# OSU-NLP-Group/saev

Hardware: AMD Instinct MI355X
Metric: activations/sec (train step), d_in=1024 x32 k=32 (higher is better)
Workload: dtype f32 (encoder: fp16 MFMA first pass with a rigorous error margin, survivors recomputed exactly in fp32; all else fp32)

## Files before the change

### saev_amd/csrc/common.h

```cpp
#pragma once
#include <hip/hip_runtime.h>
#include <stdint.h>

#define WAVE 64

typedef float f32x4 __attribute__((ext_vector_type(4)));
typedef float f32x16 __attribute__((ext_vector_type(16)));

__device__ __forceinline__ int32_t f2key(float f) {
    int32_t b = __float_as_int(f);
    return b >= 0 ? b : (b ^ 0x7fffffff);
}
__device__ __forceinline__ float key2f(int32_t k) {
    return __int_as_float(k >= 0 ? k : (k ^ 0x7fffffff));
}
__device__ __forceinline__ uint32_t f2ukey(float f) {
    uint32_t b = __float_as_uint(f);
    return (b & 0x80000000u) ? ~b : (b | 0x80000000u);
}
__device__ __forceinline__ float ukey2f(uint32_t k) {
    return __uint_as_float((k & 0x80000000u) ? (k & 0x7fffffffu) : ~k);
}

__device__ __forceinline__ float wave_sum(float v) {
#pragma unroll
    for (int o = 32; o > 0; o >>= 1) v += __shfl_xor(v, o, 64);
    return v;
}
__device__ __forceinline__ double wave_sum_d(double v) {
#pragma unroll
    for (int o = 32; o > 0; o >>= 1) v += __shfl_xor(v, o, 64);
    return v;
}
__device__ __forceinline__ int wave_sum_i(int v) {
#pragma unroll
    for (int o = 32; o > 0; o >>= 1) v += __shfl_xor(v, o, 64);
    return v;
}
__device__ __forceinline__ float wave_max(float v) {
#pragma unroll
    for (int o = 32; o > 0; o >>= 1) v = fmaxf(v, __shfl_xor(v, o, 64));
    return v;
}

#define NEG_INF (-__builtin_huge_valf())

__device__ __forceinline__ float rpg_apply(float g, float sc, float w) { return __builtin_fmaf(-sc, w, g); }
template <int NV>
__device__ __forceinline__ float rpg_row_stats(const f32x4 (&g)[NV], const f32x4 (&w)[NV], int project, float* sc_out) {
    float dot = 0.f, nsq = 0.f;
#pragma unroll
    for (int n = 0; n < NV; ++n)
#pragma unroll
        for (int e = 0; e < 4; ++e) { dot = __builtin_fmaf(g[n][e], w[n][e], dot); nsq = __builtin_fmaf(w[n][e], w[n][e], nsq); }
    dot = wave_sum(dot);
    nsq = wave_sum(nsq);
    const float sc = (project && nsq > 0.f) ? dot / nsq : 0.f;
    float sq = 0.f;
#pragma unroll
    for (int n = 0; n < NV; ++n)
#pragma unroll
        for (int e = 0; e < 4; ++e) { const float t = rpg_apply(g[n][e], sc, w[n][e]); sq = __builtin_fmaf(t, t, sq); }
    *sc_out = sc;
    return wave_sum(sq);
}
```

### saev_amd/csrc/sparse.hip

```cpp
#include "common.h"
#include "kernels.h"

namespace {

template <int NV>
__device__ __forceinline__ void gather_rows_accum(f32x4 (&acc)[NV], const float* __restrict__ W, int D, int D4,
                                                  const int32_t* idx_row, const float* val_row, int k, int limit,
                                                  int lane) {
    for (int j0 = 0; j0 < k; j0 += 64) {
        const int cnt = min(64, k - j0);
        int32_t my_i = -1;
        float my_v = 0.f;
        if (lane < cnt) { my_i = idx_row[j0 + lane]; my_v = val_row[j0 + lane]; }
#pragma unroll 4
        for (int jj = 0; jj < cnt; ++jj) {
            const int32_t i = __shfl(my_i, jj, 64);
            const float v = __shfl(my_v, jj, 64);
            if (i < 0 || i >= limit) continue;
            const f32x4* wr = reinterpret_cast<const f32x4*>(W + (size_t)i * D);
#pragma unroll
            for (int n = 0; n < NV; ++n) {
                const int q = lane + 64 * n;
                if (q < D4) {
                    const f32x4 w = wr[q];
// ... 544 lines not shown
    __syncthreads();
    int off[3] = {0, 0, 0};
    for (int j = 0; j < w; ++j)
        for (int q = 0; q < 3; ++q) off[q] += wave_tot[j][q];
    if (i < a.S) {
        a.starts[i] = off[0] + incl[0] - v[0];
        if (a.chunk_starts) {
            a.chunk_starts[i] = off[1] + incl[1] - v[1];
            a.part_starts[i] = off[2] + incl[2] - v[2];
        }
    }
    if (tid == 1023)
        for (int q = 0; q < 3; ++q) a.scan_totals[blockIdx.x * 3 + q] = off[q] + incl[q];
}
__global__ __launch_bounds__(1024) void csc_scan_offset_kernel(CscArgs a) {
    if (a.k_dev && *a.k_dev <= 0) return;
    __shared__ int base[3];
    const int tid = threadIdx.x, lane = tid & 63;
    if (tid < 64) {
        int s3[3] = {0, 0, 0};
        for (int b = lane; b < (int)blockIdx.x; b += 64)
            for (int q = 0; q < 3; ++q) s3[q] += a.scan_totals[b * 3 + q];
        for (int q = 0; q < 3; ++q) s3[q] = wave_sum_i(s3[q]);
        if (lane == 0)
            for (int q = 0; q < 3; ++q) base[q] = s3[q];
    }
    __syncthreads();
    const int i = blockIdx.x * 1024 + tid;
    if (i < a.S) {
        a.starts[i] += base[0];
        if (a.chunk_starts) { a.chunk_starts[i] += base[1]; a.part_starts[i] += base[2]; }
    }
    if (blockIdx.x == gridDim.x - 1 && tid == 0) {
        if (a.zero_word != nullptr) *a.zero_word = 0;
        a.starts[a.S] = base[0] + a.scan_totals[blockIdx.x * 3 + 0];
        if (a.chunk_starts) a.chunk_starts[a.S] = base[1] + a.scan_totals[blockIdx.x * 3 + 1];
    }
}

__global__ void csc_place_kernel(CscArgs a) {
    const int k = a.k_dev ? min(*a.k_dev, a.k) : a.k;
    if (k <= 0) return;
    const long n = (long)a.n_rows * k;
    const int groups = a.words >> 3;
    for (long p = (long)blockIdx.x * blockDim.x + threadIdx.x; p < max(n, (long)a.S); p += (long)gridDim.x * blockDim.x) {
        if (p < a.S && a.chunk_starts) {
            const int c1 = a.chunk_starts[p + 1];
            for (int c = a.chunk_starts[p]; c < c1; ++c) a.work_latent[c] = (int)p;
        }
        if (p >= n) continue;
        const int b = (int)(p / k), j = (int)(p % k);
        const int32_t i = a.idx[(size_t)b * a.code_stride + j];
        if (i < 0 || i >= a.S) continue;
        const int g = b >> 8, wi = (b >> 5) & 7;
        const uint4* grp = reinterpret_cast<const uint4*>(a.bitmap + (size_t)i * a.words + 8 * g);
        const uint4 lo = grp[0], hi = grp[1];
        const uint32_t wd[8] = {lo.x, lo.y, lo.z, lo.w, hi.x, hi.y, hi.z, hi.w};
        int rank = a.grp_prefix[(size_t)i * groups + g];
#pragma unroll
        for (int e = 0; e < 8; ++e) {
            const uint32_t m = e < wi ? 0xffffffffu : (e == wi ? ((1u << (b & 31)) - 1u) : 0u);
            rank += __popc(wd[e] & m);
        }
        const int slot = a.starts[i] + rank;
        if (a.pairs != nullptr) a.pairs[slot] = int2{b, (int)((size_t)b * a.code_stride + j)};
        if (a.pv != nullptr) {
            const int fl = (rank == 0 ? DWS_FIRST : 0) | (rank == a.counts[i] - 1 ? DWS_LAST : 0);
            int pblk = 0;
            if (a.P > 1) while (pblk < a.P - 1 && i >= a.cuts[pblk]) ++pblk;
            a.pv[slot] = int2{((pblk * a.n_rows + b) << 7) | fl, __float_as_int(a.val[(size_t)b * a.code_stride + j])};
            a.plat[slot] = i;
            if (a.pv2 != nullptr) a.pv2[slot] = int2{(b << 7) | fl, __float_as_int(a.dval[(size_t)b * a.code_stride + j])};
        }
    }
}


template <int NV>
__device__ __forceinline__ void write_row_proj(float2* row_proj, int i, const f32x4 (&g)[NV], const f32x4 (&w)[NV], int project,
                                               int lane) {
    float sc;
    const float sq = rpg_row_stats<NV>(g, w, project, &sc);
    if (lane == 0) row_proj[i] = float2{sc, sq};
}

template <int NV>
__device__ __forceinline__ float row_sumsq(const f32x4 (&g)[NV]) {
    float sq = 0.f;
#pragma unroll
    for (int n = 0; n < NV; ++n)
#pragma unroll
        for (int e = 0; e < 4; ++e) sq = __builtin_fmaf(g[n][e], g[n][e], sq);
    return wave_sum(sq);
}

#ifndef DW_MIN_WAVES
#define DW_MIN_WAVES 1
#endif
#ifndef DW_GROUP
#define DW_GROUP 8
#endif
template <int NV>
__global__ __launch_bounds__(256, DW_MIN_WAVES) void dw_rows_kernel(DwRowsArgs a) {
    if (a.k_dev && *a.k_dev <= 0) return;
    const int lane = threadIdx.x & 63;
    const int wi = a.chunk_starts[a.lat_lo] + blockIdx.x * 4 + (threadIdx.x >> 6);
    const int n_work = a.chunk_starts[a.lat_hi];
    if (wi >= n_work) return;
    const int i = a.work_latent[wi];
    const int c = wi - a.chunk_starts[i];
    const int nch = a.chunk_starts[i + 1] - a.chunk_starts[i];
    const int D = a.D, D4 = D >> 2;
    const int seg_beg = a.starts[i], seg_end = a.starts[i + 1];
    int pblk = 0;
    if (a.P > 1) while (pblk < a.P - 1 && i >= a.cuts[pblk]) ++pblk;
    const size_t g_stride = (size_t)a.P * D;
    const float* gbase = a.g + (size_t)pblk * D;
    const int beg = seg_beg + c * DW_CHUNK;
    const int end = min(seg_end, beg + DW_CHUNK);
    f32x4 accd[NV], acce[NV], wv[NV];
    {
        const f32x4* wr = reinterpret_cast<const f32x4*>(a.W_dec + (size_t)i * D);
#pragma unroll
        for (int n = 0; n < NV; ++n) {
            accd[n] = f32x4{0.f, 0.f, 0.f, 0.f};
            acce[n] = f32x4{0.f, 0.f, 0.f, 0.f};
            wv[n] = (a.part != 2 && lane + 64 * n < D4) ? wr[lane + 64 * n] : f32x4{0.f, 0.f, 0.f, 0.f};
        }
    }
    int my_b = 0;
    float my_v = 0.f, my_dv = 0.f;
    const int cnt = end - beg;
    const int part = a.part;
    if (lane < cnt) {
        const int2 pr = a.pairs[beg + lane];
        my_b = pr.x;
        my_v = a.val[pr.y];
        if (part == 2) my_dv = a.dval[beg + lane];
        if (a.clear_bitmap != nullptr) a.clear_bitmap[(size_t)i * a.clear_words + (my_b >> 5)] = 0u;
    }
    float dbs = 0.f;
    constexpr int G = DW_GROUP, GS = (G == 8 ? 3 : 4);
    for (int j0 = 0; j0 < cnt; j0 += G) {
        float p[G];
        float r = 0.f;
        if (part != 2) {
#pragma unroll
        for (int t = 0; t < G; t += 2) {
            p[t] = 0.f; p[t + 1] = 0.f;
            if (j0 + t >= cnt) continue;
            const bool two = j0 + t + 1 < cnt;
            const int b0 = __shfl(my_b, j0 + t, 64), b1 = __shfl(my_b, min(j0 + t + 1, 63), 64);
            const float v0 = __shfl(my_v, j0 + t, 64), v1 = two ? __shfl(my_v, min(j0 + t + 1, 63), 64) : 0.f;
            const f32x4* g0 = reinterpret_cast<const f32x4*>(gbase + (size_t)b0 * g_stride);
            const f32x4* g1 = reinterpret_cast<const f32x4*>(gbase + (size_t)(two ? b1 : b0) * g_stride);
            f32x4 tg0[NV], tg1[NV];
#pragma unroll
            for (int n = 0; n < NV; ++n) {
                const int q = lane + 64 * n;
                const bool ok = q < D4;
                tg0[n] = ok ? g0[q] : f32x4{0.f, 0.f, 0.f, 0.f};
                tg1[n] = ok ? g1[q] : f32x4{0.f, 0.f, 0.f, 0.f};
            }
#pragma unroll
            for (int n = 0; n < NV; ++n) {
                accd[n] += v0 * tg0[n];
                accd[n] += v1 * tg1[n];
                p[t] += tg0[n][0] * wv[n][0] + tg0[n][1] * wv[n][1] + tg0[n][2] * wv[n][2] + tg0[n][3] * wv[n][3];
                p[t + 1] += tg1[n][0] * wv[n][0] + tg1[n][1] * wv[n][1] + tg1[n][2] * wv[n][2] + tg1[n][3] * wv[n][3];
            }
            if (!two) p[t + 1] = 0.f;
        }
        r = wave_reduce_scatter<G>(p, lane);
        if (part == 1) {
            if ((lane & ((1 << GS) - 1)) == 0 && j0 + (lane >> GS) < cnt) a.dval[beg + j0 + (lane >> GS)] = r;
            continue;
        }
        }
#pragma unroll
        for (int t = 0; t < G; t += 2) {
            if (j0 + t >= cnt) continue;
            const bool two = j0 + t + 1 < cnt;
            const float e0 = part == 2 ? __shfl(my_dv, j0 + t, 64) : __shfl(r, t << GS, 64);
            const float e1 = !two ? 0.f : part == 2 ? __shfl(my_dv, min(j0 + t + 1, 63), 64) : __shfl(r, (t + 1) << GS, 64);
            dbs += e0 + e1;
            const int b0 = __shfl(my_b, j0 + t, 64), b1 = __shfl(my_b, min(j0 + t + 1, 63), 64);
            const f32x4* x0 = reinterpret_cast<const f32x4*>(a.x + (size_t)b0 * D);
            const f32x4* x1 = reinterpret_cast<const f32x4*>(a.x + (size_t)(two ? b1 : b0) * D);
            f32x4 tx0[NV], tx1[NV];
#pragma unroll
            for (int n = 0; n < NV; ++n) {
                const int q = lane + 64 * n;
                const bool ok = q < D4;
                tx0[n] = ok ? x0[q] : f32x4{0.f, 0.f, 0.f, 0.f};
                tx1[n] = ok ? x1[q] : f32x4{0.f, 0.f, 0.f, 0.f};
            }
#pragma unroll
            for (int n = 0; n < NV; ++n) {
                acce[n] += e0 * tx0[n];
                acce[n] += e1 * tx1[n];
            }
        }
    }

    float *od, *oe;
    bool direct = (nch == 1);
    if (direct) {
        od = a.dW_dec + (size_t)i * D;
        oe = a.dW_encT + (size_t)i * D;
    } else {
        od = a.partials + (size_t)(a.part_starts[i] + c) * 2 * D;
        oe = od + D;
    }
#pragma unroll
    for (int n = 0; n < NV; ++n) {
        const int q = lane + 64 * n;
        if (q < D4) {
            f32x4* pd = reinterpret_cast<f32x4*>(od) + q;
            f32x4* pe = reinterpret_cast<f32x4*>(oe) + q;
            if (part != 2) { if (direct && a.accumulate) *pd = *pd + accd[n]; else *pd = accd[n]; }
            if (part != 1) { if (direct && a.accumulate) *pe = *pe + acce[n]; else *pe = acce[n]; }
        }
    }
    if (lane == 0 && part != 1) {
        if (direct) a.db_enc[i] = a.accumulate ? (a.db_enc[i] + dbs) : dbs;
        else a.db_partials[a.part_starts[i] + c] = dbs;
    }
    if (a.row_proj != nullptr && direct && part != 2 && !a.accumulate) write_row_proj<NV>(a.row_proj, i, accd, wv, a.project, lane);
    if (a.enc_sq != nullptr && direct && part != 1 && !a.accumulate) {
        const float sq = row_sumsq<NV>(acce);
        if (lane == 0) a.enc_sq[i] = sq;
    }
}

template <int NV>
__global__ __launch_bounds__(256) void dw_combine_kernel(DwRowsArgs a) {
    if (a.k_dev && *a.k_dev <= 0) return;
    const int lane = threadIdx.x & 63;
    const int i = a.lat_lo + blockIdx.x * 4 + (threadIdx.x >> 6);
    if (i >= a.lat_hi) return;
    const int enc = blockIdx.y;
    if ((enc == 0 && a.part == 2) || (enc == 1 && a.part == 1)) return;
    const int nch = a.chunk_starts[i + 1] - a.chunk_starts[i];
    if (nch <= 1) return;
    const int c0 = a.part_starts[i], c1 = c0 + nch;
    const int D = a.D, D4 = D >> 2;
    const float* base = a.partials + (enc ? D : 0);
    f32x4 acc[NV];
#pragma unroll
    for (int n = 0; n < NV; ++n) acc[n] = f32x4{0.f, 0.f, 0.f, 0.f};
    float dbs = 0.f;
    int c = c0;
    constexpr int TRIP = NV <= 4 ? 8 : (NV <= 8 ? 4 : 2);
    for (; c + TRIP <= c1; c += TRIP) {
        f32x4 t[TRIP][NV];
#pragma unroll
        for (int u = 0; u < TRIP; ++u) {
            const f32x4* p = reinterpret_cast<const f32x4*>(base + (size_t)(c + u) * 2 * D);
#pragma unroll
            for (int n = 0; n < NV; ++n) t[u][n] = (lane + 64 * n < D4) ? p[lane + 64 * n] : f32x4{0.f, 0.f, 0.f, 0.f};
        }
#pragma unroll
        for (int n = 0; n < NV; ++n) {
            if constexpr (TRIP == 8) acc[n] += ((t[0][n] + t[1][n]) + (t[2][n] + t[3][n])) + ((t[4][n] + t[5][n]) + (t[6][n] + t[7][n]));
            else if constexpr (TRIP == 4) acc[n] += (t[0][n] + t[1][n]) + (t[2][n] + t[3][n]);
            else acc[n] += t[0][n] + t[1][n];
        }
        if (enc) {
#pragma unroll
            for (int u = 0; u < TRIP; ++u) dbs += a.db_partials[c + u];
        }
    }
    for (; c < c1; ++c) {
        const f32x4* p = reinterpret_cast<const f32x4*>(base + (size_t)c * 2 * D);
#pragma unroll
        for (int n = 0; n < NV; ++n)
            if (lane + 64 * n < D4) acc[n] += p[lane + 64 * n];
        if (enc) dbs += a.db_partials[c];
    }
    f32x4* o = reinterpret_cast<f32x4*>((enc ? a.dW_encT : a.dW_dec) + (size_t)i * D);
#pragma unroll
    for (int n = 0; n < NV; ++n) {
        const int q = lane + 64 * n;
        if (q < D4) o[q] = a.accumulate ? o[q] + acc[n] : acc[n];
    }
    if (enc) {
        if (lane == 0) a.db_enc[i] = a.accumulate ? (a.db_enc[i] + dbs) : dbs;
        if (a.enc_sq != nullptr && !a.accumulate) {
            const float sq = row_sumsq<NV>(acc);
            if (lane == 0) a.enc_sq[i] = sq;
        }
    } else if (a.row_proj != nullptr && !a.accumulate) {
        f32x4 wv[NV];
        const f32x4* wr = reinterpret_cast<const f32x4*>(a.W_dec + (size_t)i * D);
#pragma unroll
        for (int n = 0; n < NV; ++n) wv[n] = (lane + 64 * n < D4) ? wr[lane + 64 * n] : f32x4{0.f, 0.f, 0.f, 0.f};
        write_row_proj<NV>(a.row_proj, i, acc, wv, a.project, lane);
    }
}


typedef int i32x2 __attribute__((ext_vector_type(2)));
typedef int i32x4 __attribute__((ext_vector_type(4)));

__device__ __forceinline__ f32x4 buf_load16(__amdgpu_buffer_rsrc_t r, uint32_t voff) {
    const i32x4 v = __builtin_amdgcn_raw_buffer_load_b128(r, voff, 0, 0);
    return f32x4{__int_as_float(v[0]), __int_as_float(v[1]), __int_as_float(v[2]), __int_as_float(v[3])};
}
__device__ __forceinline__ float group8_sum(float v) {
    v += __int_as_float(__builtin_amdgcn_mov_dpp(__float_as_int(v), 0xB1, 0xF, 0xF, true));
    v += __int_as_float(__builtin_amdgcn_mov_dpp(__float_as_int(v), 0x4E, 0xF, 0xF, true));
    v += __int_as_float(__builtin_amdgcn_mov_dpp(__float_as_int(v), 0x141, 0xF, 0xF, true));
    return v;
}

__global__ __launch_bounds__(256) void slice_major_copy_kernel(const float* __restrict__ g, const float* __restrict__ x, int n, int D,
                                                               float* __restrict__ gS, float* __restrict__ xS) {
    const int lane = threadIdx.x & 63;
    const int row = blockIdx.x * 4 + (threadIdx.x >> 6);
    if (row >= n) return;
    const f32x4* gr = reinterpret_cast<const f32x4*>(g + (size_t)row * D);
    const f32x4* xr = reinterpret_cast<const f32x4*>(x + (size_t)row * D);
    for (int q = lane; q < (D >> 2); q += 64) {
        const size_t o = ((size_t)(q >> 3) * n + row) * 8 + (q & 7);
        reinterpret_cast<f32x4*>(gS)[o] = gr[q];
        reinterpret_cast<f32x4*>(xS)[o] = xr[q];
    }
}

template <bool DEC, bool DVAL = true>
__global__ __launch_bounds__(256, (DEC && DVAL) ? 4 : 5) void dw_slices_kernel(DwSlicesArgs a, int wg_per_slice) {
    constexpr bool PASS_A = DEC && DVAL;
    constexpr int L = DWS_RUN;
    const int lane = threadIdx.x & 63, gi = lane >> 3, li = lane & 7;
    const int xcd = blockIdx.x & 7, q = blockIdx.x >> 3;
    const int slice = xcd + 8 * (q / wg_per_slice);
    const bool sq_on = (DEC ? a.sq_wave_dec : a.sq_wave_enc) != nullptr;
    auto sq_slot = [&]() -> float* {
        return (DEC ? a.sq_wave_dec : a.sq_wave_enc) + ((size_t)blockIdx.x * 4 + __builtin_amdgcn_readfirstlane((int)(threadIdx.x >> 6)));
    };
    if (slice * DWS_SLICE >= a.D) { if (sq_on && lane == 0) *sq_slot() = 0.f; return; }
    const int NP = a.starts[a.S];
    const int run0 = ((q % wg_per_slice) * 4 + (threadIdx.x >> 6)) * 8;
    if (run0 * L >= NP) { if (sq_on && lane == 0) *sq_slot() = 0.f; return; }
    const int run = run0 + gi;
    const int col = slice * DWS_SLICE + li * 4;
    const uint32_t colb = (uint32_t)col * 4u, rowb = (uint32_t)a.D * 4u, li16 = (uint32_t)li * 16u;
    auto bound = [&](int r) -> int {
        const long nb = (long)r * L;
        if (nb >= NP) return NP;
        const int lat = a.plat[nb];
        const int s = a.starts[lat];
        return (a.starts[lat + 1] - s < L) ? s : (int)nb;
    };
    const int p0 = bound(run), p1 = bound(run + 1);
    const bool live = p0 < p1;
    const int2* const pv = DEC ? a.pv : a.pv2;
    float* const out = DEC ? a.dW_dec : a.dW_encT;
    float* const part = DEC ? a.part_dec : a.part_enc;
    f32x4 acc = {0.f, 0.f, 0.f, 0.f};
    f32x4 w4 = {0.f, 0.f, 0.f, 0.f};
    float* const dvp = PASS_A ? a.dvp + (size_t)slice * a.pair_cap : nullptr;
    __shared__ float sh_sq[256];
    sh_sq[threadIdx.x] = 0.f;
    const int sel = (lane & 56) << 2;
    const __amdgpu_buffer_rsrc_t mres = __builtin_amdgcn_make_buffer_rsrc(
        const_cast<float*>(DEC ? a.gS : a.xS) + (size_t)slice * a.n_rows * DWS_SLICE * (DEC && a.P > 1 ? a.P : 1), 0,
        (uint32_t)a.n_rows * 128u * (uint32_t)(DEC && a.P > 1 ? a.P : 1), 0x00020000);
    const __amdgpu_buffer_rsrc_t wres = __builtin_amdgcn_make_buffer_rsrc(const_cast<float*>(a.W_dec), 0, (uint32_t)a.S * rowb, 0x00020000);

    auto load_info = [&](int t, int2& e, int& lat) {
        const int p = p0 + 8 * t + li;
        e = int2{0, 0};
        lat = 0;
        if (p < p1) {
            const i32x2 v = reinterpret_cast<const i32x2*>(pv)[p];
            e = int2{v[0], v[1]};
            lat = a.plat[p];
            if (p == p1 - 1) e.x |= DWS_END;
            if (p == p0) e.x &= ~DWS_FIRST;
        }
    };
    constexpr int PB = 4;
    auto issue = [&](const int2& e, int lat, int j0, int (&xj)[PB], int (&lj)[PB], f32x4 (&gt)[PB], f32x4 (&wt)[PB]) {
#pragma unroll
        for (int j = 0; j < PB; ++j) {
            xj[j] = __builtin_amdgcn_ds_bpermute(sel + 4 * (j0 + j), e.x);
            lj[j] = __builtin_amdgcn_ds_bpermute(sel + 4 * (j0 + j), lat);
            gt[j] = buf_load16(mres, ((uint32_t)xj[j] & ~127u) | li16);
            if (PASS_A && (xj[j] & DWS_FIRST)) wt[j] = buf_load16(wres, (uint32_t)lj[j] * rowb + colb);
        }
    };
    auto consume = [&](const int2& e, int j0, const int (&xc)[PB], const int (&lc)[PB], const f32x4 (&gc)[PB], const f32x4 (&wc)[PB],
                       const f32x4& wnext0, bool& head_open, float& dmine) {
        float vc[PB];
#pragma unroll
        for (int j = 0; j < PB; ++j) vc[j] = __int_as_float(__builtin_amdgcn_ds_bpermute(sel + 4 * (j0 + j), e.y));
#pragma unroll
        for (int j = 0; j < PB; ++j) {
            if (PASS_A) {
                float d = gc[j][0] * w4[0] + gc[j][1] * w4[1] + gc[j][2] * w4[2] + gc[j][3] * w4[3];
                d = group8_sum(d);
                dmine = li == j0 + j ? d : dmine;
            }
            acc += vc[j] * gc[j];
            if (xc[j] & (DWS_LAST | DWS_END)) {
                float* o;
                if (head_open) o = part + ((size_t)run * 2 + 0) * a.D + col;
                else if (!(xc[j] & DWS_LAST)) o = part + ((size_t)run * 2 + 1) * a.D + col;
                else {
                    o = out + (size_t)lc[j] * a.D + col;
                    if (sq_on)
                        sh_sq[threadIdx.x] += __builtin_fmaf(acc[3], acc[3], __builtin_fmaf(acc[2], acc[2], __builtin_fmaf(acc[1], acc[1], acc[0] * acc[0])));
                }
                *reinterpret_cast<f32x4*>(o) = acc;
                if (DEC && slice == 0 && li == 0 && (xc[j] & DWS_END)) {
                    const int cl = (!head_open && !(xc[j] & DWS_LAST)) ? lc[j] : -1;
                    a.cut_lat[run] = cl;
                    if (cl >= 0 && a.cut_list != nullptr)
                        reinterpret_cast<i32x4*>(a.cut_list)[1 + atomicAdd(&a.cut_list[0], 1)] = i32x4{run, cl, a.starts[cl], a.starts[cl + 1]};
                }
                head_open = false;
                acc = f32x4{0.f, 0.f, 0.f, 0.f};
                if (PASS_A) w4 = j + 1 < PB ? wc[j + 1 < PB ? j + 1 : 0] : wnext0;
            }
        }
    };
    int2 e_c, e_n;
    int lat_c, lat_n;
    int xa[PB], xb[PB], la[PB], lb[PB];
    f32x4 ga[PB], gb[PB], wa[PB], wb[PB];
    bool head_open = false;
    load_info(0, e_c, lat_c);
    if (live) {
        head_open = (pv[p0].x & DWS_FIRST) == 0;
        if (PASS_A) w4 = buf_load16(wres, (uint32_t)a.plat[p0] * rowb + colb);
    }
    issue(e_c, lat_c, 0, xa, la, ga, wa);
    load_info(1, e_n, lat_n);
#pragma unroll 1
    for (int t = 0; __any(p0 + 8 * t < p1); ++t) {
        float dmine = 0.f;
        issue(e_c, lat_c, PB, xb, lb, gb, wb);
        consume(e_c, 0, xa, la, ga, wa, wb[0], head_open, dmine);
        issue(e_n, lat_n, 0, xa, la, ga, wa);
        consume(e_c, PB, xb, lb, gb, wb, wa[0], head_open, dmine);
        if (PASS_A && p0 + 8 * t + li < p1) dvp[p0 + 8 * t + li] = dmine;
        e_c = e_n; lat_c = lat_n;
        load_info(t + 2, e_n, lat_n);
    }
    if (sq_on) {
        const float sq = wave_sum(sh_sq[threadIdx.x]);
        if (lane == 0) *sq_slot() = sq;
    }
}

__global__ __launch_bounds__(256) void dw_dval_sum_kernel(DwSlicesArgs a) {
    const int NP = a.starts[a.S];
    const int p = blockIdx.x * 256 + threadIdx.x;
    if (p >= NP) return;
    const int n_slices = a.D / DWS_SLICE;
    float s = 0.f;
    for (int c = 0; c < n_slices; ++c) s += a.dvp[(size_t)c * a.pair_cap + p];
    const int2 e = a.pv[p];
    const int b = a.P > 1 ? (e.x >> 7) % a.n_rows : (e.x >> 7);
    a.pv2[p] = int2{(b << 7) | (e.x & 127), __float_as_int(s)};
    if (a.clear_bitmap != nullptr) a.clear_bitmap[(size_t)a.plat[p] * a.clear_words + (b >> 5)] = 0u;
}

__global__ __launch_bounds__(256) void dw_clear_bitmap_kernel(DwSlicesArgs a) {
    const int NP = a.starts[a.S];
    const int p = blockIdx.x * 256 + threadIdx.x;
    if (p >= NP) return;
    a.clear_bitmap[(size_t)a.plat[p] * a.clear_words + (a.pv2[p].x >> 12)] = 0u;
}

template <int NV>
__global__ __launch_bounds__(256) void dw_finalize_cut_kernel(DwSlicesArgs a, int kind0) {
    constexpr int L = DWS_RUN;
    __shared__ f32x4 sh[3][NV * 64];
    __shared__ float shdb[4];
    const int lane = threadIdx.x & 63, w = threadIdx.x >> 6;
    const int NP = a.starts[a.S];
    const int r0 = blockIdx.x;
    if ((long)(r0 + 1) * L >= NP) return;
    const int i = a.cut_lat[r0];
    if (i < 0) return;
    const int s = a.starts[i], e = a.starts[i + 1];
    const int r1 = (e - 1) / L;
    const int enc = blockIdx.y + kind0;
    const int D = a.D, D4 = D >> 2;
    const float* const part = enc ? a.part_enc : a.part_dec;
    const int nh = r1 - r0, ch = (nh + 3) / 4;
    const int ra = r0 + 1 + w * ch, rb = min(r1 + 1, ra + ch);
    f32x4 acc[NV];
#pragma unroll
    for (int n = 0; n < NV; ++n) acc[n] = f32x4{0.f, 0.f, 0.f, 0.f};
    int r = ra;
    constexpr int TRIP = NV <= 4 ? 4 : 2;
    for (; r + TRIP <= rb; r += TRIP) {
        f32x4 t[TRIP][NV];
#pragma unroll
        for (int u = 0; u < TRIP; ++u) {
            const f32x4* p = reinterpret_cast<const f32x4*>(part + (size_t)(r + u) * 2 * D);
#pragma unroll
            for (int n = 0; n < NV; ++n) t[u][n] = (lane + 64 * n < D4) ? p[lane + 64 * n] : f32x4{0.f, 0.f, 0.f, 0.f};
        }
#pragma unroll
        for (int n = 0; n < NV; ++n) {
            if constexpr (TRIP == 4) acc[n] += (t[0][n] + t[1][n]) + (t[2][n] + t[3][n]);
            else acc[n] += t[0][n] + t[1][n];
        }
    }
    for (; r < rb; ++r) {
        const f32x4* p = reinterpret_cast<const f32x4*>(part + (size_t)r * 2 * D);
#pragma unroll
        for (int n = 0; n < NV; ++n)
            if (lane + 64 * n < D4) acc[n] += p[lane + 64 * n];
    }
    float dbs = 0.f;
    if (enc) {
        const int cnt = e - s, q4 = (cnt + 3) / 4;
        const int pend = min(e, s + (w + 1) * q4);
        for (int p0 = s + w * q4 + lane; p0 < pend; p0 += 64 * 8) {
            float t[8];
#pragma unroll
            for (int u = 0; u < 8; ++u) t[u] = (p0 + 64 * u < pend) ? __int_as_float(a.pv2[p0 + 64 * u].y) : 0.f;
#pragma unroll
            for (int u = 0; u < 8; ++u)
                if (p0 + 64 * u < pend) dbs += t[u];
        }
        dbs = wave_sum(dbs);
    }
    if (w != 0) {
#pragma unroll
        for (int n = 0; n < NV; ++n) sh[w - 1][lane + 64 * n] = acc[n];
    }
    if (lane == 0) shdb[w] = dbs;
    __syncthreads();
    if (w != 0) return;
    {
        const f32x4* p = reinterpret_cast<const f32x4*>(part + ((size_t)r0 * 2 + 1) * D);
#pragma unroll
        for (int n = 0; n < NV; ++n) {
            const f32x4 t = (lane + 64 * n < D4) ? p[lane + 64 * n] : f32x4{0.f, 0.f, 0.f, 0.f};
            acc[n] = (((t + acc[n]) + sh[0][lane + 64 * n]) + sh[1][lane + 64 * n]) + sh[2][lane + 64 * n];
        }
    }
    float* const row = (enc ? a.dW_encT : a.dW_dec) + (size_t)i * D;
#pragma unroll
    for (int n = 0; n < NV; ++n)
        if (lane + 64 * n < D4) reinterpret_cast<f32x4*>(row)[lane + 64 * n] = acc[n];
    if (enc) {
        if (lane == 0) a.db_enc[i] = ((shdb[0] + shdb[1]) + shdb[2]) + shdb[3];
        if (a.enc_sq != nullptr) {
            const float sq = row_sumsq<NV>(acc);
            if (lane == 0) a.enc_sq[i] = sq;
        }
    } else if (a.row_proj != nullptr) {
        f32x4 wv[NV];
        const f32x4* wr = reinterpret_cast<const f32x4*>(a.W_dec + (size_t)i * D);
#pragma unroll
        for (int n = 0; n < NV; ++n) wv[n] = (lane + 64 * n < D4) ? wr[lane + 64 * n] : f32x4{0.f, 0.f, 0.f, 0.f};
        write_row_proj<NV>(a.row_proj, i, acc, wv, a.project, lane);
    }
}

template <int NV>
__global__ __launch_bounds__(256) void dw_finalize_kernel(DwSlicesArgs a, int kind0) {
    constexpr int L = DWS_RUN;
    const int lane = threadIdx.x & 63;
    const int i = blockIdx.x * 4 + (threadIdx.x >> 6);
    if (i >= a.S) return;
    const int enc = blockIdx.y + kind0;
    const int D = a.D, D4 = D >> 2;
    const int s = a.starts[i], e = a.starts[i + 1];
    if (!enc && a.lat_unused != nullptr && lane == 0) a.lat_unused[i] = e == s ? 1 : 0;
    if (e - s >= L && s / L != (e - 1) / L) return;
    float* const row = (enc ? a.dW_encT : a.dW_dec) + (size_t)i * D;
    f32x4 acc[NV], wv[NV];
    const bool proj = !enc && a.row_proj != nullptr;
    const f32x4* wr = reinterpret_cast<const f32x4*>(a.W_dec + (size_t)i * D);
#pragma unroll
    for (int n = 0; n < NV; ++n) {
        acc[n] = f32x4{0.f, 0.f, 0.f, 0.f};
        wv[n] = f32x4{0.f, 0.f, 0.f, 0.f};
        if (lane + 64 * n < D4) {
            if (e > s) acc[n] = reinterpret_cast<const f32x4*>(row)[lane + 64 * n];
            else if (!(enc && a.lat_unused != nullptr)) reinterpret_cast<f32x4*>(row)[lane + 64 * n] = acc[n];
            if (proj) wv[n] = wr[lane + 64 * n];
        }
    }
    if (enc) {
        float dbs = 0.f;
        for (int p = s + lane; p < e; p += 64) dbs += __int_as_float(a.pv2[p].y);
        dbs = wave_sum(dbs);
        if (lane == 0) a.db_enc[i] = dbs;
        if (a.enc_sq != nullptr) {
            const float sq = row_sumsq<NV>(acc);
            if (lane == 0) a.enc_sq[i] = sq;
        }
    } else if (proj) {
        write_row_proj<NV>(a.row_proj, i, acc, wv, a.project, lane);
    }
}

template <int NV>
__global__ __launch_bounds__(256) void dw_finalize_light_kernel(DwSlicesArgs a, int n_cut_blocks) {
    constexpr int L = DWS_RUN;
    __shared__ f32x4 sh[3][NV * 64];
    __shared__ float shdb[4];
    const int lane = threadIdx.x & 63, w = threadIdx.x >> 6;
    const int D = a.D, D4 = D >> 2;
    if ((int)blockIdx.x < n_cut_blocks) {
      const i32x4 first = reinterpret_cast<const i32x4*>(a.cut_list)[1 + (blockIdx.x >> 1)];
      const int n_items = 2 * a.cut_list[0];
      for (int item = blockIdx.x; item < n_items; item += n_cut_blocks) {
        const i32x4 ent = item == (int)blockIdx.x ? first : reinterpret_cast<const i32x4*>(a.cut_list)[1 + (item >> 1)];
        const int r0 = ent[0], i = ent[1], s = ent[2], e = ent[3], enc = item & 1;
        const int r1 = (e - 1) / L;
        const float* const part = enc ? a.part_enc : a.part_dec;
        f32x4 tp[NV], wv[NV];
        if (w == 0) {
            const f32x4* p = reinterpret_cast<const f32x4*>(part + ((size_t)r0 * 2 + 1) * D);
            const f32x4* wr = reinterpret_cast<const f32x4*>(a.W_dec + (size_t)i * D);
            const bool need_w = !enc && a.row_proj != nullptr;
#pragma unroll
            for (int n = 0; n < NV; ++n) {
                const bool ok = lane + 64 * n < D4;
                tp[n] = ok ? p[lane + 64 * n] : f32x4{0.f, 0.f, 0.f, 0.f};
                wv[n] = (ok && need_w) ? wr[lane + 64 * n] : f32x4{0.f, 0.f, 0.f, 0.f};
            }
        }
        const int nh = r1 - r0, ch = (nh + 3) / 4;
        const int ra = r0 + 1 + w * ch, rb = min(r1 + 1, ra + ch);
        f32x4 acc[NV];
#pragma unroll
        for (int n = 0; n < NV; ++n) acc[n] = f32x4{0.f, 0.f, 0.f, 0.f};
        constexpr int TRIP = NV <= 4 ? 4 : 2;
        int r = ra;
        for (; r + 2 * TRIP <= rb; r += 2 * TRIP) {
            f32x4 t[2 * TRIP][NV];
#pragma unroll
            for (int u = 0; u < 2 * TRIP; ++u) {
                const f32x4* p = reinterpret_cast<const f32x4*>(part + (size_t)(r + u) * 2 * D);
#pragma unroll
                for (int n = 0; n < NV; ++n) t[u][n] = (lane + 64 * n < D4) ? p[lane + 64 * n] : f32x4{0.f, 0.f, 0.f, 0.f};
            }
#pragma unroll
            for (int n = 0; n < NV; ++n) {
                if constexpr (TRIP == 4) {
                    acc[n] += (t[0][n] + t[1][n]) + (t[2][n] + t[3][n]);
                    acc[n] += (t[4][n] + t[5][n]) + (t[6][n] + t[7][n]);
                } else {
                    acc[n] += t[0][n] + t[1][n];
                    acc[n] += t[2][n] + t[3][n];
                }
            }
        }
        for (; r + TRIP <= rb; r += TRIP) {
            f32x4 t[TRIP][NV];
#pragma unroll
            for (int u = 0; u < TRIP; ++u) {
                const f32x4* p = reinterpret_cast<const f32x4*>(part + (size_t)(r + u) * 2 * D);
#pragma unroll
                for (int n = 0; n < NV; ++n) t[u][n] = (lane + 64 * n < D4) ? p[lane + 64 * n] : f32x4{0.f, 0.f, 0.f, 0.f};
            }
#pragma unroll
            for (int n = 0; n < NV; ++n) {
                if constexpr (TRIP == 4) acc[n] += (t[0][n] + t[1][n]) + (t[2][n] + t[3][n]);
                else acc[n] += t[0][n] + t[1][n];
            }
        }
        for (; r < rb; ++r) {
            const f32x4* p = reinterpret_cast<const f32x4*>(part + (size_t)r * 2 * D);
#pragma unroll
            for (int n = 0; n < NV; ++n)
                if (lane + 64 * n < D4) acc[n] += p[lane + 64 * n];
        }
        float dbs = 0.f;
        if (enc) {
            const int cnt = e - s, q4 = (cnt + 3) / 4;
            const int pend = min(e, s + (w + 1) * q4);
            for (int p0 = s + w * q4 + lane; p0 < pend; p0 += 64 * 8) {
                int2 pe[8];
#pragma unroll
                for (int u = 0; u < 8; ++u) pe[u] = (p0 + 64 * u < pend) ? a.pv2[p0 + 64 * u] : int2{0, 0};
#pragma unroll
                for (int u = 0; u < 8; ++u) {
                    if (p0 + 64 * u < pend) {
                        dbs += __int_as_float(pe[u].y);
                        if (a.clear_bitmap != nullptr) a.clear_bitmap[(size_t)i * a.clear_words + (pe[u].x >> 12)] = 0u;
                    }
                }
            }
            dbs = wave_sum(dbs);
        }
        if (w != 0) {
#pragma unroll
            for (int n = 0; n < NV; ++n) sh[w - 1][lane + 64 * n] = acc[n];
        }
        if (lane == 0) shdb[w] = dbs;
        __syncthreads();
        if (w == 0) {
#pragma unroll
            for (int n = 0; n < NV; ++n) acc[n] = (((tp[n] + acc[n]) + sh[0][lane + 64 * n]) + sh[1][lane + 64 * n]) + sh[2][lane + 64 * n];
            float* const row = (enc ? a.dW_encT : a.dW_dec) + (size_t)i * D;
#pragma unroll
            for (int n = 0; n < NV; ++n)
                if (lane + 64 * n < D4) reinterpret_cast<f32x4*>(row)[lane + 64 * n] = acc[n];
            if (enc) {
                if (lane == 0) a.db_enc[i] = ((shdb[0] + shdb[1]) + shdb[2]) + shdb[3];
                if (a.enc_sq != nullptr) {
                    const float sq = row_sumsq<NV>(acc);
                    if (lane == 0) a.enc_sq[i] = sq;
                }
            } else if (a.row_proj != nullptr) {
                write_row_proj<NV>(a.row_proj, i, acc, wv, a.project, lane);
            }
        }
        __syncthreads();
      }
      return;
    }
    const int li = lane & 7;
    const int i = ((int)blockIdx.x - n_cut_blocks) * 32 + (int)(threadIdx.x >> 3);
    if (i >= a.S) return;
    const int s = a.starts[i], e = a.starts[i + 1];
    if (a.lat_unused != nullptr && li == 0) a.lat_unused[i] = e == s ? 1 : 0;
    if (e - s >= L && s / L != (e - 1) / L) return;
    if (e == s) {
        if (a.lat_unused == nullptr) {
            for (int q = li; q < D4; q += 8) {
                reinterpret_cast<f32x4*>(a.dW_dec + (size_t)i * D)[q] = f32x4{0.f, 0.f, 0.f, 0.f};
                reinterpret_cast<f32x4*>(a.dW_encT + (size_t)i * D)[q] = f32x4{0.f, 0.f, 0.f, 0.f};
            }
        }
        if (li == 0) {
            a.db_enc[i] = 0.f;
            if (a.enc_sq != nullptr) a.enc_sq[i] = 0.f;
            if (a.row_proj != nullptr) a.row_proj[i] = float2{0.f, 0.f};
        }
        return;
    }
    auto group_tree = [&](float (&v)[8]) -> float {
        float r = ((v[0] + v[4]) + (v[2] + v[6])) + ((v[1] + v[5]) + (v[3] + v[7]));
        r += __shfl_xor(r, 4, 64);
        r += __shfl_xor(r, 2, 64);
        r += __shfl_xor(r, 1, 64);
        return r;
    };
    float gsq = 0.f, esq = 0.f;
// ... 432 lines not shown
```

Baseline: 6.291 million.

## Broadcast pair metadata via DPP row_newbcast and load two pairs per lane

Each lane in the dW slice kernel now loads two consecutive (index, value) pairs and their latent ids with a single wider load, and the main loop covers 16 pairs per iteration instead of 8. The ds_bpermute broadcasts inside each 8-lane group are replaced with DPP update_dpp row broadcasts, which avoid the LDS crossbar path. The occupancy hint for the pass-A variant also drops from 4 to 3 waves per SIMD, giving the longer unrolled loop more registers. Risks are higher register pressure, lower occupancy hiding less latency, and misaligned vector loads when pair offsets are odd.

```diff
diff --git a/saev_amd/csrc/common.h b/saev_amd/csrc/common.h
--- a/saev_amd/csrc/common.h
+++ b/saev_amd/csrc/common.h
@@ -43,6 +43,25 @@
     return v;
 }
 
+template <int U>
+__device__ __forceinline__ int group8_bcast(int v) {
+    static_assert(U >= 0 && U < 8, "a group has eight lanes");
+    const int r = __builtin_amdgcn_update_dpp(0, v, 0x150 + U, 0xF, 0x3, false);
+    return __builtin_amdgcn_update_dpp(r, v, 0x150 + 8 + U, 0xF, 0xC, false);
+}
+__device__ __forceinline__ int group8_bcast(int v, int u) {
+    switch (u & 7) {
+        case 0: return group8_bcast<0>(v);
+        case 1: return group8_bcast<1>(v);
+        case 2: return group8_bcast<2>(v);
+        case 3: return group8_bcast<3>(v);
+        case 4: return group8_bcast<4>(v);
+        case 5: return group8_bcast<5>(v);
+        case 6: return group8_bcast<6>(v);
+        default: return group8_bcast<7>(v);
+    }
+}
+
 #define NEG_INF (-__builtin_huge_valf())
 
 __device__ __forceinline__ float rpg_apply(float g, float sc, float w) { return __builtin_fmaf(-sc, w, g); }
diff --git a/saev_amd/csrc/sparse.hip b/saev_amd/csrc/sparse.hip
--- a/saev_amd/csrc/sparse.hip
+++ b/saev_amd/csrc/sparse.hip
@@ -870,6 +870,8 @@
 
 typedef int i32x2 __attribute__((ext_vector_type(2)));
 typedef int i32x4 __attribute__((ext_vector_type(4)));
+typedef i32x4 i32x4_a8 __attribute__((aligned(8)));
+typedef i32x2 i32x2_a4 __attribute__((aligned(4)));
 
 __device__ __forceinline__ f32x4 buf_load16(__amdgpu_buffer_rsrc_t r, uint32_t voff) {
     const i32x4 v = __builtin_amdgcn_raw_buffer_load_b128(r, voff, 0, 0);
@@ -896,8 +898,11 @@
     }
 }
 
+#ifndef DWS_PASS_A_WAVES
+#define DWS_PASS_A_WAVES 3
+#endif
 template <bool DEC, bool DVAL = true>
-__global__ __launch_bounds__(256, (DEC && DVAL) ? 4 : 5) void dw_slices_kernel(DwSlicesArgs a, int wg_per_slice) {
+__global__ __launch_bounds__(256, (DEC && DVAL) ? DWS_PASS_A_WAVES : 5) void dw_slices_kernel(DwSlicesArgs a, int wg_per_slice) {
     constexpr bool PASS_A = DEC && DVAL;
     constexpr int L = DWS_RUN;
     const int lane = threadIdx.x & 63, gi = lane >> 3, li = lane & 7;
@@ -931,45 +936,55 @@
     float* const dvp = PASS_A ? a.dvp + (size_t)slice * a.pair_cap : nullptr;
     __shared__ float sh_sq[256];
     sh_sq[threadIdx.x] = 0.f;
-    const int sel = (lane & 56) << 2;
     const __amdgpu_buffer_rsrc_t mres = __builtin_amdgcn_make_buffer_rsrc(
         const_cast<float*>(DEC ? a.gS : a.xS) + (size_t)slice * a.n_rows * DWS_SLICE * (DEC && a.P > 1 ? a.P : 1), 0,
         (uint32_t)a.n_rows * 128u * (uint32_t)(DEC && a.P > 1 ? a.P : 1), 0x00020000);
     const __amdgpu_buffer_rsrc_t wres = __builtin_amdgcn_make_buffer_rsrc(const_cast<float*>(a.W_dec), 0, (uint32_t)a.S * rowb, 0x00020000);
 
-    auto load_info = [&](int t, int2& e, int& lat) {
-        const int p = p0 + 8 * t + li;
-        e = int2{0, 0};
-        lat = 0;
-        if (p < p1) {
-            const i32x2 v = reinterpret_cast<const i32x2*>(pv)[p];
-            e = int2{v[0], v[1]};
-            lat = a.plat[p];
-            if (p == p1 - 1) e.x |= DWS_END;
-            if (p == p0) e.x &= ~DWS_FIRST;
+    auto load_info = [&](int T, i32x4& v, i32x2& l) {
+        const int p = p0 + 16 * T + 2 * li;
+        v = i32x4{0, 0, 0, 0};
+        l = i32x2{0, 0};
+        if (p + 1 < p1) {
+            v = *reinterpret_cast<const i32x4_a8*>(pv + p);
+            l = *reinterpret_cast<const i32x2_a4*>(a.plat + p);
+        } else if (p < p1) {
+            const i32x2 t = reinterpret_cast<const i32x2*>(pv)[p];
+            v = i32x4{t[0], t[1], 0, 0};
+            l = i32x2{a.plat[p], 0};
         }
     };
+    auto finish_info = [&](int T, const i32x4& v, i32x4& e) {
+        const int p = p0 + 16 * T + 2 * li;
+        e = v;
+        if (p == p1 - 1) e[0] |= DWS_END;
+        if (p + 1 == p1 - 1) e[2] |= DWS_END;
+        if (p == p0) e[0] &= ~DWS_FIRST;
+    };
+    auto pair_x = [&](const i32x4& e, int u) -> int { return group8_bcast((u & 1) ? e[2] : e[0], u >> 1); };
+    auto pair_v = [&](const i32x4& e, int u) -> float { return __int_as_float(group8_bcast((u & 1) ? e[3] : e[1], u >> 1)); };
+    auto pair_l = [&](const i32x2& l, int u) -> int { return group8_bcast((u & 1) ? l[1] : l[0], u >> 1); };
     constexpr int PB = 4;
-    auto issue = [&](const int2& e, int lat, int j0, int (&xj)[PB], int (&lj)[PB], f32x4 (&gt)[PB], f32x4 (&wt)[PB]) {
+    auto issue = [&](const i32x4& e, const i32x2& l, int sb, int (&xj)[PB], int (&lj)[PB], f32x4 (&gt)[PB], f32x4 (&wt)[PB]) {
 #pragma unroll
         for (int j = 0; j < PB; ++j) {
-            xj[j] = __builtin_amdgcn_ds_bpermute(sel + 4 * (j0 + j), e.x);
-            lj[j] = __builtin_amdgcn_ds_bpermute(sel + 4 * (j0 + j), lat);
+            xj[j] = pair_x(e, 4 * sb + j);
+            lj[j] = pair_l(l, 4 * sb + j);
             gt[j] = buf_load16(mres, ((uint32_t)xj[j] & ~127u) | li16);
             if (PASS_A && (xj[j] & DWS_FIRST)) wt[j] = buf_load16(wres, (uint32_t)lj[j] * rowb + colb);
         }
     };
-    auto consume = [&](const int2& e, int j0, const int (&xc)[PB], const int (&lc)[PB], const f32x4 (&gc)[PB], const f32x4 (&wc)[PB],
+    auto consume = [&](const i32x4& e, int sb, const int (&xc)[PB], const int (&lc)[PB], const f32x4 (&gc)[PB], const f32x4 (&wc)[PB],
                        const f32x4& wnext0, bool& head_open, float& dmine) {
         float vc[PB];
 #pragma unroll
-        for (int j = 0; j < PB; ++j) vc[j] = __int_as_float(__builtin_amdgcn_ds_bpermute(sel + 4 * (j0 + j), e.y));
+        for (int j = 0; j < PB; ++j) vc[j] = pair_v(e, 4 * sb + j);
 #pragma unroll
         for (int j = 0; j < PB; ++j) {
             if (PASS_A) {
                 float d = gc[j][0] * w4[0] + gc[j][1] * w4[1] + gc[j][2] * w4[2] + gc[j][3] * w4[3];
                 d = group8_sum(d);
-                dmine = li == j0 + j ? d : dmine;
+                dmine = li == ((4 * sb + j) & 7) ? d : dmine;
             }
             acc += vc[j] * gc[j];
             if (xc[j] & (DWS_LAST | DWS_END)) {
@@ -994,28 +1009,39 @@
             }
         }
     };
-    int2 e_c, e_n;
-    int lat_c, lat_n;
+    i32x4 rv, e_c, e_n;
+    i32x2 rl, l_c, l_n;
     int xa[PB], xb[PB], la[PB], lb[PB];
     f32x4 ga[PB], gb[PB], wa[PB], wb[PB];
     bool head_open = false;
-    load_info(0, e_c, lat_c);
+    load_info(0, rv, rl);
+    finish_info(0, rv, e_c);
+    l_c = rl;
     if (live) {
         head_open = (pv[p0].x & DWS_FIRST) == 0;
         if (PASS_A) w4 = buf_load16(wres, (uint32_t)a.plat[p0] * rowb + colb);
     }
-    issue(e_c, lat_c, 0, xa, la, ga, wa);
-    load_info(1, e_n, lat_n);
+    issue(e_c, l_c, 0, xa, la, ga, wa);
+    load_info(1, rv, rl);
 #pragma unroll 1
-    for (int t = 0; __any(p0 + 8 * t < p1); ++t) {
+    for (int T = 0; __any(p0 + 16 * T < p1); ++T) {
+        const int pb = p0 + 16 * T;
         float dmine = 0.f;
-        issue(e_c, lat_c, PB, xb, lb, gb, wb);
+        issue(e_c, l_c, 1, xb, lb, gb, wb);
         consume(e_c, 0, xa, la, ga, wa, wb[0], head_open, dmine);
-        issue(e_n, lat_n, 0, xa, la, ga, wa);
-        consume(e_c, PB, xb, lb, gb, wb, wa[0], head_open, dmine);
-        if (PASS_A && p0 + 8 * t + li < p1) dvp[p0 + 8 * t + li] = dmine;
-        e_c = e_n; lat_c = lat_n;
-        load_info(t + 2, e_n, lat_n);
+        issue(e_c, l_c, 2, xa, la, ga, wa);
+        consume(e_c, 1, xb, lb, gb, wb, wa[0], head_open, dmine);
+        if (PASS_A && pb + li < p1) dvp[pb + li] = dmine;
+        dmine = 0.f;
+        issue(e_c, l_c, 3, xb, lb, gb, wb);
+        consume(e_c, 2, xa, la, ga, wa, wb[0], head_open, dmine);
+        finish_info(T + 1, rv, e_n);
+        l_n = rl;
+        issue(e_n, l_n, 0, xa, la, ga, wa);
+        consume(e_c, 3, xb, lb, gb, wb, wa[0], head_open, dmine);
+        if (PASS_A && pb + 8 + li < p1) dvp[pb + 8 + li] = dmine;
+        e_c = e_n; l_c = l_n;
+        load_info(T + 2, rv, rl);
     }
     if (sq_on) {
         const float sq = wave_sum(sh_sq[threadIdx.x]);
```

After: 6.276 million. No clear change (-0.2%).
